# NVIDIA/nvidia-resiliency-ext

Measured on AMD Instinct MI355X. Metric: generate_report_latency_us, lower is better.
Workload: dtype f32; 1 GPU; 8 ranks x 64 sections x 10000 samples per report, ring capacity 10000, relative+individual scores, gather_on_rank0; logical_ranks_per_gpu=8, rows_per_gpu=512, exchange=none (single process)

## Files before the change

### include/nvrx_straggler.h

```cpp
#ifndef NVRX_STRAGGLER_H
#define NVRX_STRAGGLER_H

#include <stddef.h>
#include <stdint.h>

#ifdef __cplusplus
extern "C" {
#endif

#define NVRX_ABI_VERSION 2

#define NVRX_OK 0
#define NVRX_ERR_INVALID (-22)
#define NVRX_ERR_NOMEM (-12)
#define NVRX_ERR_HIP (-5)
#define NVRX_ERR_STATE (-1)
#define NVRX_ERR_RANGE (-34)
#define NVRX_ERR_TIMEOUT (-62)

#define NVRX_STATS_STRIDE 8
#define NVRX_STAT_MIN 0
#define NVRX_STAT_MAX 1
#define NVRX_STAT_MED 2
#define NVRX_STAT_AVG 3
// ... 11 lines not shown
#define NVRX_SCORE_LEN(S) (2 + 2 * (S))
#define NVRX_META_WORDS 8

typedef struct nvrx_ctx nvrx_ctx;

int nvrx_abi_version(void);
const char *nvrx_last_error(void);


int nvrx_row_stats(const float *d_samples, const uint32_t *d_counts, const uint8_t *d_kinds, int rows,
                   int row_stride, float *d_stats, void *stream);

int nvrx_score(const float *d_table, int R, int K, int S, int do_indiv, int do_rel,
               const double *thresholds, float *d_scores, uint8_t *d_flags, uint32_t *d_meta,
               uint32_t *d_done_counter, uint32_t seq, const float *d_stats_src, float *d_stats_dst,
               int stats_rows, void *stream);

#define NVRX_SCORE_ROUTE_SINGLE 1
#define NVRX_SCORE_ROUTE_ROWS 2
#define NVRX_SCORE_ROUTE_ROWS_PRE 3
#define NVRX_SCORE_ROUTE_TILE16 4
#define NVRX_SCORE_ROUTE_TILE8 5
int nvrx_score_route(int R, int K, int S, const void *d_scores, const void *d_flags);

#define NVRX_ATTR_MAX_TOP 16
#define NVRX_ATTR_SCRATCH_FLOATS(K) (33 * (size_t)(K))
#define NVRX_ATTR_WORDS(n_ranks, top_n) ((size_t)(n_ranks) * 2 * (1 + (size_t)(top_n)) * 4)
int nvrx_attribute(const float *d_table, int R, int K, int S, int first_rank, int n_ranks, int top_n, int do_indiv,
                   int do_rel, float *d_minmed_scratch, void *d_out, void *stream);

int nvrx_row_quantile(const float *d_samples, const uint32_t *d_counts, int rows, int row_stride, uint32_t q_ppm,
                      float *d_out, void *stream);
int nvrx_tail_score(const float *d_tails, const float *d_table, int R, int K, int S, int first_rank, int n_ranks,
                    float *d_colmin_scratch, float *d_out, void *stream);

int nvrx_row_onset(const float *d_samples, const uint32_t *d_counts, const uint32_t *d_starts, int rows, int row_stride,
                   uint32_t min_seg_ppm, void *d_out, void *stream);
#define NVRX_ONSET_PLANES 6
int nvrx_onset_score(const float *d_onset, const float *d_table, int R, int K, int S, int first_rank, int n_ranks,
                     float *d_colmin_scratch, float *d_out, void *stream);

#define NVRX_PERIOD_MIN_CYCLES 4
#define NVRX_PERIOD_MAX 4096
#define NVRX_PERIOD_BAR 0.95
int nvrx_row_period(const float *d_samples, const uint32_t *d_counts, const uint32_t *d_starts, int rows, int row_stride,
                    int max_period, void *d_out, void *stream);
// ... 212 lines not shown
```

### nvidia-resiliency-ext_amd/csrc/nvrx_straggler.hip

```cpp
#include <hip/hip_runtime.h>
#include <hip/hip_ext.h>

#include <algorithm>
#include <atomic>
#include <chrono>
#include <thread>
#include <cmath>
#include <cstdarg>
#include <cstdio>
#include <cstdlib>
#include <cstring>
#include <deque>
#include <mutex>
#include <string>
#include <unordered_map>
#include <utility>
#include <vector>

#include "nvrx_straggler.h"

namespace {

thread_local std::string g_err;

// ... 21 lines not shown
    g_report_clk[i] = std::chrono::duration<double, std::micro>(std::chrono::steady_clock::now().time_since_epoch()).count();
}

__device__ __forceinline__ uint32_t f2key(float f) {
    uint32_t u = __float_as_uint(f);
    return u ^ ((u >> 31) ? 0xFFFFFFFFu : 0x80000000u);
}
__device__ __forceinline__ float key2f(uint32_t k) {
    uint32_t u = (k & 0x80000000u) ? (k ^ 0x80000000u) : ~k;
    return __uint_as_float(u);
}

typedef float f32x2 __attribute__((ext_vector_type(2)));

template <int CTRL, int ROW_MASK = 0xf>
__device__ __forceinline__ uint32_t dpp(uint32_t old, uint32_t src) {
    return (uint32_t)__builtin_amdgcn_update_dpp((int)old, (int)src, CTRL, ROW_MASK, 0xf, false);
}
template <int CTRL>
__device__ __forceinline__ uint32_t dpp0(uint32_t src) {
    return (uint32_t)__builtin_amdgcn_update_dpp(0, (int)src, CTRL, 0xf, 0xf, true);
}
constexpr int DPP_QUAD_1032 = 0xb1, DPP_QUAD_2301 = 0x4e, DPP_ROW_SHR1 = 0x111, DPP_ROW_SHR2 = 0x112,
              DPP_ROW_SHR4 = 0x114, DPP_ROW_SHR8 = 0x118, DPP_BCAST15 = 0x142, DPP_BCAST31 = 0x143;

__device__ __forceinline__ uint32_t wave_min_u32(uint32_t v) {
    v = min(v, dpp<DPP_QUAD_1032>(0xFFFFFFFFu, v));
    v = min(v, dpp<DPP_QUAD_2301>(0xFFFFFFFFu, v));
    v = min(v, dpp<DPP_ROW_SHR4>(0xFFFFFFFFu, v));
    v = min(v, dpp<DPP_ROW_SHR8>(0xFFFFFFFFu, v));
    v = min(v, dpp<DPP_BCAST15>(0xFFFFFFFFu, v));
    v = min(v, dpp<DPP_BCAST31>(0xFFFFFFFFu, v));
    return (uint32_t)__builtin_amdgcn_readlane((int)v, 63);
}
__device__ __forceinline__ uint32_t wave_max_u32(uint32_t v) {
    v = max(v, dpp0<DPP_QUAD_1032>(v));
    v = max(v, dpp0<DPP_QUAD_2301>(v));
    v = max(v, dpp0<DPP_ROW_SHR4>(v));
    v = max(v, dpp0<DPP_ROW_SHR8>(v));
    v = max(v, dpp0<DPP_BCAST15>(v));
    v = max(v, dpp0<DPP_BCAST31>(v));
    return (uint32_t)__builtin_amdgcn_readlane((int)v, 63);
}
__device__ __forceinline__ uint32_t wave_sum_u32(uint32_t v) {
    v += dpp0<DPP_QUAD_1032>(v);
    v += dpp0<DPP_QUAD_2301>(v);
    v += dpp0<DPP_ROW_SHR4>(v);
// ... 1142 lines not shown
    }
}

__global__ __launch_bounds__(PEER_THREADS) void k_peer_allgather(PeerArgs a) { peer_exchange_block(a); }

constexpr int SCORE1_THREADS = 1024;
constexpr int SCORE1_RESIDENT_THREADS = 256;
constexpr int SCORE1_MAX_RANKS = 64;
constexpr size_t SCORE1_MAX_LDS = 60 * 1024;

__device__ __forceinline__ void store16_sys(void *dst, nvrx_f4 v) {
    asm volatile("global_store_dwordx4 %0, %1, off sc0 sc1" : : "v"(dst), "v"(v) : "memory");
}

__host__ __device__ inline size_t score1_lds_bytes(int R, int K, int S) {
    const size_t ks4 = (size_t)((K + S + 3) & ~3);
    const size_t nout = (size_t)R * NVRX_SCORE_LEN(S);
    return ks4 * 4 + ((nout + 3) & ~(size_t)3) * 4 + ((nout + 15) & ~(size_t)15);
}
__host__ __device__ inline size_t score1_table_lds_bytes(int R, int K, int S, int send_floats) {
    return (((size_t)R * NVRX_TABLE_LEN(K, S) + 3) & ~(size_t)3) * 4 + (((size_t)send_floats + 3) & ~(size_t)3) * 4;
}

struct GatherArgs {
    const unsigned long long *g;
    const int32_t *gid;
    float *send;
    nvrx_f4 *stats_out;
    uint32_t *err;
    int n_blocks, rows_active, rows_per_rank, local_ranks;
    float names_ok;
    uint32_t epoch;
    unsigned long long timeout_ticks;
    int poll_naps;
};

__device__ __forceinline__ float wait_granule(const unsigned long long *p, const GatherArgs &g, unsigned long long t0) {
    uint32_t spins = 0;
    for (;;) {
        const unsigned long long x = __hip_atomic_load(p, __ATOMIC_RELAXED, __HIP_MEMORY_SCOPE_AGENT);
        if ((uint32_t)(x >> 32) == g.epoch) return __uint_as_float((uint32_t)x);
        __builtin_amdgcn_s_sleep(2);
        if ((++spins & 0xFFu) == 0u && wall_clock64() - t0 > g.timeout_ticks) {
            __hip_atomic_store(g.err, g.epoch, __ATOMIC_RELAXED, __HIP_MEMORY_SCOPE_SYSTEM);
            return __builtin_nanf("");
        }
    }
}

template <int NTHR>
__global__ __launch_bounds__(NTHR) void k_score1(ScoreArgs a, int fence, PeerArgs pa, GatherArgs ga) {
    extern __shared__ __attribute__((aligned(16))) unsigned char s_raw[];

    const int K = a.K, S = a.S, KS = K + S, R = a.R;
    const int L = NVRX_TABLE_LEN(K, S);
    const int W = NVRX_SCORE_LEN(S);
    const int nout = R * W;
    const int nout4 = (nout + 3) & ~3;
    float *s_min = reinterpret_cast<float *>(s_raw);
    float *s_out = s_min + ((KS + 3) & ~3);
    uint8_t *s_fl = reinterpret_cast<uint8_t *>(s_out + nout4);
    float *s_tab = a.tab_in_lds ? reinterpret_cast<float *>(s_fl + ((nout + 15) & ~15)) : nullptr;
    float *s_send = a.tab_in_lds ? s_tab + ((R * L + 3) & ~3) : nullptr;
    const int tid = threadIdx.x;
    const float NaN = __builtin_nanf("");
    const unsigned long long t_begin = wall_clock64();
#if NVRX_TOUCH_KERNARGS
    {
        constexpr int KARG_DWORDS = (int)((sizeof(ScoreArgs) + sizeof(int) + sizeof(PeerArgs) + sizeof(GatherArgs)) / 4);
        const uint32_t __attribute__((address_space(4))) *ka =
// ... 1 lines not shown
        uint32_t touched = 0u;
#pragma unroll
        for (int d = 0; d < KARG_DWORDS; d += 16) touched ^= ka[d];
        asm volatile("" ::"s"(touched));
    }
#endif
    const int pair_r0 = tid / max(S, 1), pair_s0 = tid - pair_r0 * S;
    const int pair_dr = NTHR / max(S, 1), pair_ds = NTHR - pair_dr * S;
    const bool lds_only = ga.g && s_send;
    auto sync = [&]() {
        if (lds_only)
            asm volatile("s_waitcnt lgkmcnt(0)\n\ts_barrier" ::: "memory");
        else
            __syncthreads();
    };

    if (ga.g && s_send) {
        for (int j = tid; j < a.send_floats; j += NTHR) {
            const int col = j % L;
            s_send[j] = col < KS ? -1.0f : (col < 2 * KS ? NaN : 0.0f);
        }
        __syncthreads();
    }
    if (ga.g) {
        constexpr int CH = 8;
        const int total = ga.n_blocks * 3;
        for (int base = tid; base < total; base += NTHR * CH) {
            unsigned long long x[CH];
            int slot[CH];
            uint32_t pending = 0;
#pragma unroll
            for (int c = 0; c < CH; c++) {
                slot[c] = -1;
                const int idx = base + c * NTHR;
                if (idx < total) {
                    pending |= 1u << c;
                    const int b = idx / 3, q = idx - 3 * b;
                    const int lr = b / ga.rows_active;
                    const int gidv = ga.gid[lr * ga.rows_per_rank + (b - lr * ga.rows_active)];
                    if (gidv >= 0 && gidv < KS && (q < 2 || gidv < K)) slot[c] = lr * L + q * KS + gidv;
                }
            }
            uint32_t spins = 0;
            while (pending) {
#pragma unroll
                for (int c = 0; c < CH; c++)
                    if (pending & (1u << c)) {
// ... 9 lines not shown
                    if (!got && (spins & 0xFFu) == 0xFFu && wall_clock64() - t_begin > ga.timeout_ticks) {
                        __hip_atomic_store(ga.err, ga.epoch, __ATOMIC_RELAXED, __HIP_MEMORY_SCOPE_SYSTEM);
                        v = NaN;
                        got = true;
                    }
                    if (got) {
                        if (slot[c] >= 0) {
                            ga.send[slot[c]] = v;
                            if (s_send) s_send[slot[c]] = v;
                        }
                        pending &= ~(1u << c);
                    }
                }
                if (pending) {
                    for (int nap = 0; nap < ga.poll_naps; nap++) __builtin_amdgcn_s_sleep(1);
                    spins++;
                }
            }
        }
        for (int lr = tid; lr < ga.local_ranks; lr += NTHR) {
            ga.send[(size_t)lr * L + (L - 1)] = ga.names_ok;
            if (s_send) s_send[lr * L + (L - 1)] = ga.names_ok;
        }
        sync();
    }
    const unsigned long long t_rows = wall_clock64();
    if (pa.windows) {
        peer_exchange_block(pa, ga.g ? s_send : nullptr, s_tab);
        __syncthreads();
        if (s_tab) a.table = s_tab;
    } else if (ga.g && s_send) {
        a.table = s_send;
    }
    for (int i = tid; i < a.stats_n4; i += NTHR) {
        const float4 v = a.stats_src[i];
        store16_sys(a.stats_dst + i, nvrx_f4{v.x, v.y, v.z, v.w});
    }
    auto score_all = [&](const float *tab) {
        score_colmin(a, tab, tid, NTHR, s_min);
        if (a.meta && (tid >> 6) == NTHR / 64 - 1) score_meta(a, tab, tid & 63);
        if (tid < nout4 - nout) s_out[nout + tid] = 0.f;
        if (tid < ((nout + 15) & ~15) - nout) s_fl[nout + tid] = 0;
        sync();

        {
            int r = pair_r0, sct = pair_s0;
#pragma unroll 2
            for (int idx = tid; idx < R * S; idx += NTHR) {
                const float *__restrict__ row = tab + (size_t)r * L;
                const float med = row[K + sct];
                float si = NaN, sr = NaN;
                if (med >= 0.0f) {
                    if (a.do_indiv) si = __fdiv_rn(row[KS + K + sct], med);
                    if (a.do_rel) sr = __fdiv_rn(s_min[K + sct], med);
                }
                s_out[r * W + 2 + sct] = si;
                s_out[r * W + 2 + S + sct] = sr;
                s_fl[r * W + 2 + sct] = ((double)si < a.thr[3]) ? 1 : 0;
                s_fl[r * W + 2 + S + sct] = ((double)sr < a.thr[1]) ? 1 : 0;
                r += pair_dr;
                sct += pair_ds;
                if (sct >= S) {
                    sct -= S;
                    r++;
                }
            }
        }
        if (K == 0) {
            for (int r = tid; r < R; r += NTHR) {
                s_out[r * W] = NaN;
                s_out[r * W + 1] = NaN;
                s_fl[r * W] = 0;
                s_fl[r * W + 1] = 0;
            }
        } else {
            const int lane = tid & 63;
            for (int r = tid >> 6; r < R; r += NTHR / 64) {
                const float *__restrict__ row = tab + (size_t)r * L;
                double wi = 0.0, si = 0.0, wr = 0.0, sr = 0.0;
                uint32_t nk = 0, ncommon = 0;
                for (int k = lane; k < K; k += 64) {
                    const float medf = row[k];
                    if (!(medf >= 0.0f)) continue;
                    const double med = (double)medf;
                    const double w = (double)row[2 * KS + k];
                    nk++;
                    si += ((double)row[KS + k] / med) * w;
                    wi += w;
                    const float mm = s_min[k];
                    if (mm == mm) {
                        ncommon++;
                        sr += ((double)mm / med) * w;
                        wr += w;
                    }
                }
                wi = wave_sum_f64(wi);
                si = wave_sum_f64(si);
                wr = wave_sum_f64(wr);
                sr = wave_sum_f64(sr);
                nk = wave_sum_u32(nk);
                ncommon = wave_sum_u32(ncommon);
                if (lane == 0) {
                    const float gi = (a.do_indiv && nk > 0) ? (float)(si / wi) : NaN;
                    const float gr = (a.do_rel && ncommon > 0) ? (float)(sr / wr) : NaN;
                    s_out[r * W] = gi;
                    s_out[r * W + 1] = gr;
                    s_fl[r * W] = ((double)gi < a.thr[2]) ? 1 : 0;
                    s_fl[r * W + 1] = ((double)gr < a.thr[0]) ? 1 : 0;
                }
            }
        }
        sync();
    };
    if (s_tab && pa.windows)
        score_all(s_tab);
    else if (ga.g && s_send && !pa.windows)
        score_all(s_send);
    else
        score_all(a.table);

    const unsigned long long t_staged = wall_clock64();
    {
        const nvrx_f4 *src = reinterpret_cast<const nvrx_f4 *>(s_out);
        nvrx_f4 *dst = reinterpret_cast<nvrx_f4 *>(a.scores);
        for (int i = tid; i < nout4 / 4; i += NTHR) store16_sys(dst + i, src[i]);
        if (a.flags) {
            const nvrx_f4 *fsrc = reinterpret_cast<const nvrx_f4 *>(s_fl);
            nvrx_f4 *fdst = reinterpret_cast<nvrx_f4 *>(a.flags);
            for (int i = tid; i < (nout + 15) / 16; i += NTHR) store16_sys(fdst + i, fsrc[i]);
        }
    }
    asm volatile("s_waitcnt vmcnt(0)" ::: "memory");
    __syncthreads();
    const bool publish = a.meta && a.done_counter;
    if (tid == 0 && publish) {
        if (fence) {
            __builtin_amdgcn_fence(__ATOMIC_RELEASE, "");
            asm volatile("s_waitcnt vmcnt(0)" ::: "memory");
        }
        if (!(ga.g && ga.stats_out))
            __hip_atomic_store(&a.meta[5], a.seq, __ATOMIC_RELAXED, __HIP_MEMORY_SCOPE_SYSTEM);
        __hip_atomic_store(&a.meta[6], (uint32_t)(t_rows - t_begin), __ATOMIC_RELAXED, __HIP_MEMORY_SCOPE_SYSTEM);
        __hip_atomic_store(&a.meta[7], (uint32_t)min(wall_clock64() - t_rows, 0xFFFFull) | ((uint32_t)min(t_staged - t_rows, 0xFFFFull) << 16),
                           __ATOMIC_RELAXED, __HIP_MEMORY_SCOPE_SYSTEM);
// ... 75 lines not shown

constexpr int score_single_wg_enabled() { return 1; }
int score_fence_enabled() {
    static int v = -1;
    if (v < 0) {
        const char *e = getenv("NVRX_DEBUG_SCORE_FENCE");
        if (e && *e) {
            v = atoi(e) != 0 ? 1 : 0;
        } else {
            int dev = 0;
            hipDeviceProp_t prop;
            v = 1;
            if (hipGetDevice(&dev) == hipSuccess && hipGetDeviceProperties(&prop, dev) == hipSuccess &&
                (strncmp(prop.gcnArchName, "gfx950", 6) == 0 || strncmp(prop.gcnArchName, "gfx942", 6) == 0))
                v = 0;
        }
    }
    return v;
}

int resident_scorer_mode_from_env() {
    const char *e = getenv("NVRX_DEBUG_RESIDENT_SCORER");
    const int v = e ? atoi(e) : 1;
    return (v < 0 || v > 2) ? 1 : v;
}
constexpr int poll_naps_from_env() {
    return 4;
}

constexpr int peer_prologue_enabled() { return 1; }

struct ScoreScratch {
    float *ptr = nullptr;
    size_t elems = 0;
};
std::mutex g_scratch_mu;
std::unordered_map<void *, ScoreScratch> g_scratch_by_stream;

}

struct EventPair {
    hipEvent_t start = nullptr;
    hipEvent_t end = nullptr;
};

struct StageBuf {
    uint32_t *h_counts = nullptr;
// ... 335 lines not shown
    Epilogue ep{};
    return launch_row_stats(d_samples, d_counts, d_kinds, rows, row_stride, d_stats, ep, as_stream(stream));
}

static bool score_fits_single_wg(int R, int K, int S, const float *d_scores, const uint8_t *d_flags) {
    return R <= SCORE1_MAX_RANKS && score1_lds_bytes(R, K, S) <= SCORE1_MAX_LDS &&
           (reinterpret_cast<uintptr_t>(d_scores) & 15u) == 0 && (reinterpret_cast<uintptr_t>(d_flags) & 15u) == 0 &&
           score_single_wg_enabled();
}

constexpr size_t SCORE_ROWS_MAX_LDS = 48 * 1024;

static int score_route(int R, int K, int S, const float *d_scores, const uint8_t *d_flags) {
    if (score_fits_single_wg(R, K, S, d_scores, d_flags)) return NVRX_SCORE_ROUTE_SINGLE;
    if (R <= 64 && (size_t)(K + S) * sizeof(float) <= SCORE_ROWS_MAX_LDS) return NVRX_SCORE_ROUTE_ROWS;
    const bool aligned = ((reinterpret_cast<uintptr_t>(d_scores) | reinterpret_cast<uintptr_t>(d_flags)) & 15u) == 0;
    if (aligned && R > 64) {
        if (score_tile_lds_bytes(16, S) <= TILE_MAX_LDS) return NVRX_SCORE_ROUTE_TILE16;
        if (score_tile_lds_bytes(8, S) <= TILE_MAX_LDS) return NVRX_SCORE_ROUTE_TILE8;
    }
    return NVRX_SCORE_ROUTE_ROWS_PRE;
}

static int score_launch(const float *d_table, int R, int K, int S, int do_indiv, int do_rel, const double *thresholds,
                        float *d_scores, uint8_t *d_flags, uint32_t *d_meta, uint32_t *d_done_counter, uint32_t seq,
                        const float *d_stats_src, float *d_stats_dst, int stats_rows, void *stream, const PeerArgs *pa,
                        const GatherArgs *ga = nullptr) {
    if (R <= 0 || K < 0 || S < 0) return fail(NVRX_ERR_INVALID, "bad table shape R=%d K=%d S=%d", R, K, S);
    if (!d_table || !d_scores) return fail(NVRX_ERR_INVALID, "null device pointer");
    hipStream_t st = as_stream(stream);
    ScoreArgs a{};
    a.table = d_table;
    a.R = R;
    a.K = K;
    a.S = S;
    a.do_indiv = do_indiv;
    a.do_rel = do_rel;
    for (int i = 0; i < 4; i++) a.thr[i] = thresholds ? thresholds[i] : 0.75;
    a.scores = d_scores;
    a.flags = d_flags;
    a.meta = d_meta;
    a.done_counter = d_meta ? d_done_counter : nullptr;
    a.seq = seq;
    if (d_stats_src && d_stats_dst && stats_rows > 0) {
        a.stats_src = reinterpret_cast<const float4 *>(d_stats_src);
        a.stats_dst = reinterpret_cast<float4 *>(d_stats_dst);
        a.stats_n4 = stats_rows * (NVRX_STATS_STRIDE / 4);
    }
    const int KS = K + S;
    const int route = score_route(R, K, S, d_scores, d_flags);
    if (route == NVRX_SCORE_ROUTE_SINGLE) {
        PeerArgs none{};
        GatherArgs nog{};
        size_t lds1 = score1_lds_bytes(R, K, S);
        if (ga || pa) {
            const int send_floats = pa ? pa->count : R * NVRX_TABLE_LEN(K, S);
            const size_t extra = score1_table_lds_bytes(R, K, S, send_floats);
            if (lds1 + extra <= SCORE1_MAX_LDS) {
                a.tab_in_lds = 1;
                a.send_floats = send_floats;
                lds1 += extra;
            }
        }
        if (ga) {
            a.stats_n4 = 0;
            hipLaunchKernelGGL(k_score1<SCORE1_RESIDENT_THREADS>, dim3(1), dim3(SCORE1_RESIDENT_THREADS), lds1, st, a,
                               score_fence_enabled(), pa ? *pa : none, *ga);
        } else {
            report_clk(7);
            hipLaunchKernelGGL(k_score1<SCORE1_THREADS>, dim3(1), dim3(SCORE1_THREADS), lds1, st, a, score_fence_enabled(),
                               pa ? *pa : none, nog);
        }
        HIP_TRY(hipGetLastError());
        return NVRX_OK;
    }
    if (ga) return fail(NVRX_ERR_STATE, "the resident scorer needs the single-workgroup score kernel");
    if (pa) return fail(NVRX_ERR_STATE, "the exchange prologue needs the single-workgroup score kernel");
    if (route != NVRX_SCORE_ROUTE_ROWS) {
        const int chunks = std::max(1, std::min(COLMIN_MAX_CHUNKS, (R + 63) / 64));
        const int rows_per_chunk = (R + chunks - 1) / chunks;
        const size_t need = (size_t)KS * (size_t)(chunks + 1);
        float *scratch = nullptr;
        {
            std::lock_guard<std::mutex> lk(g_scratch_mu);
            ScoreScratch &sc = g_scratch_by_stream[stream];
            if (sc.elems < need) {
                if (sc.ptr) HIP_TRY(hipFree(sc.ptr));
                sc = ScoreScratch{};
                HIP_TRY(hipMalloc(reinterpret_cast<void **>(&sc.ptr), std::max<size_t>(need, 1024) * sizeof(float)));
                sc.elems = std::max<size_t>(need, 1024);
// ... 15 lines not shown
        hipLaunchKernelGGL(k_score, dim3(R), dim3(SCORE_THREADS), (size_t)KS * sizeof(float), st, a);
        break;
    case NVRX_SCORE_ROUTE_ROWS_PRE:
        hipLaunchKernelGGL(k_score, dim3(R), dim3(SCORE_THREADS), 0, st, a);
        break;
    case NVRX_SCORE_ROUTE_TILE16:
    case NVRX_SCORE_ROUTE_TILE8: {
        const int tile_ranks = route == NVRX_SCORE_ROUTE_TILE16 ? 16 : 8;
        hipLaunchKernelGGL(k_score_tile, dim3((R + tile_ranks - 1) / tile_ranks), dim3(TILE_THREADS),
                           score_tile_lds_bytes(tile_ranks, S), st, a, tile_ranks);
        break;
    }
    default:
        return fail(NVRX_ERR_STATE, "no score kernel for route %d", route);
    }
    HIP_TRY(hipGetLastError());
    return NVRX_OK;
}

int nvrx_score_route(int R, int K, int S, const void *d_scores, const void *d_flags) {
    if (R <= 0 || K < 0 || S < 0) return fail(NVRX_ERR_INVALID, "bad table shape R=%d K=%d S=%d", R, K, S);
    return score_route(R, K, S, static_cast<const float *>(d_scores), static_cast<const uint8_t *>(d_flags));
}

int nvrx_score(const float *d_table, int R, int K, int S, int do_indiv, int do_rel, const double *thresholds,
               float *d_scores, uint8_t *d_flags, uint32_t *d_meta, uint32_t *d_done_counter, uint32_t seq,
               const float *d_stats_src, float *d_stats_dst, int stats_rows, void *stream) {
    return score_launch(d_table, R, K, S, do_indiv, do_rel, thresholds, d_scores, d_flags, d_meta, d_done_counter, seq,
                        d_stats_src, d_stats_dst, stats_rows, stream, nullptr);
}

int nvrx_send_init(float *d_send, int rows, int K, int S, void *stream) {
    if (!d_send || rows <= 0 || K < 0 || S < 0) return fail(NVRX_ERR_INVALID, "bad arguments");
    const size_t n = (size_t)rows * NVRX_TABLE_LEN(K, S);
    hipLaunchKernelGGL(k_send_init, dim3((unsigned)((n + 255) / 256)), dim3(256), 0, as_stream(stream), d_send, rows, K, S);
    HIP_TRY(hipGetLastError());
    return NVRX_OK;
}

int nvrx_ctx_create(int device, int local_ranks, int rows_per_rank, int ring_cap, nvrx_ctx **out) {
    if (!out) return fail(NVRX_ERR_INVALID, "out is null");
    *out = nullptr;
    if (local_ranks <= 0 || rows_per_rank <= 0 || ring_cap <= 0) return fail(NVRX_ERR_INVALID, "sizes must be positive");
    if (ring_cap > NVRX_MAX_RING_CAP) return fail(NVRX_ERR_RANGE, "ring_cap %d > %d", ring_cap, NVRX_MAX_RING_CAP);
    if ((long long)local_ranks * rows_per_rank > NVRX_MAX_ROWS) return fail(NVRX_ERR_RANGE, "too many rows");
    int ndev = 0;
// ... 858 lines not shown
        }
    }
    if (!rehomed && d->order_after_enabled && d->order_after_stream != stream) {
        std::lock_guard<std::mutex> lk(ctx->mu);
        HIP_TRY(hipEventRecord(ctx->order_ev, as_stream(d->order_after_stream)));
        HIP_TRY(hipStreamWaitEvent(as_stream(stream), ctx->order_ev, 0));
    }
    report_clk(1);
    if (d->R > 64) {
        std::lock_guard<std::mutex> lk(ctx->mu);
        if (std::find(ctx->report_streams.begin(), ctx->report_streams.end(), as_stream(stream)) == ctx->report_streams.end())
            ctx->report_streams.push_back(as_stream(stream));
    }
    const int rows_launch = (d->rows_active > 0 ? d->rows_active : ctx->rows_per_rank) * ctx->local_ranks;
    const bool peer_route = exchanging && d->allgather_fn == reinterpret_cast<void *>(&nvrx_peer_allgather) && peer_prologue_enabled();
    bool cross_stream = rehomed || (d->order_after_enabled && d->order_after_stream != stream);
    {
        std::lock_guard<std::mutex> lk(ctx->mu);
        cross_stream = cross_stream || !ctx->stamp_streams.empty();
    }
    const int rmode = ctx->resident_mode;
    const bool resident = d->resident && d->h_seq_word && !d->guard_rings && (!exchanging || peer_route) && rows_launch > 0 &&
                          score_fits_single_wg(d->R, d->K, d->S, d->d_scores, d->d_flags) &&
                          (rmode == 2 || (rmode == 1 && !cross_stream));
    if (resident) {
        {
            std::lock_guard<std::mutex> lk(ctx->mu);
            HIP_TRY(hipSetDevice(ctx->device));
            if (!ctx->score_stream) {
                bool high = true;
                const char *pe = getenv("NVRX_STREAM_PRIORITY");
                if (pe && *pe) {
                    high = !(pe[0] == 'n' || pe[0] == 'N' || pe[0] == '0' || pe[0] == 'o' || pe[0] == 'O');
                } else {
                    for (const char *var : {"WORLD_SIZE", "SLURM_NTASKS", "OMPI_COMM_WORLD_SIZE", "PMI_SIZE"}) {
                        const char *v = getenv(var);
                        if (!v || !*v) continue;
                        const long n = strtol(v, nullptr, 10);
                        if (n > 1) high = false;
                        if (n > 1 || strcmp(var, "WORLD_SIZE") == 0) break;
                    }
                }
                if (high) {
                    int least = 0, greatest = 0;
                    HIP_TRY(hipDeviceGetStreamPriorityRange(&least, &greatest));
                    HIP_TRY(hipStreamCreateWithPriority(&ctx->score_stream, hipStreamNonBlocking, greatest));
                } else {
// ... 6 lines not shown
                int orc = order_after_stamps(ctx, as_stream(stream), ctx->score_stream);
                if (orc) return orc;
            }
        }
        ctx->gran_epoch = (ctx->gran_epoch % 0x7FFFFFFFu) + 1u;
        unsigned long long *slice = ctx->d_rowg + (size_t)(ctx->gran_epoch & 1u) * (size_t)ctx->rows * ROW_GRANULES;
        int rc2 = report_local_impl(ctx, d->d_stats, d->d_send, d->K, d->S, d->names_ok, d->rows_active, stream, slice,
                                    ctx->gran_epoch);
        if (rc2) return rc2;
        GatherArgs ga{};
        ga.g = slice;
        ga.gid = ctx->d_gid;
        ga.send = d->d_send;
        ga.stats_out = (d->d_stats_dst && d->stats_rows > 0) ? reinterpret_cast<nvrx_f4 *>(d->d_stats_dst) : nullptr;
        ga.err = ctx->d_gather_err;
        ga.n_blocks = rows_launch;
        ga.rows_active = d->rows_active > 0 ? d->rows_active : ctx->rows_per_rank;
        ga.rows_per_rank = ctx->rows_per_rank;
        ga.local_ranks = ctx->local_ranks;
        ga.names_ok = d->names_ok ? 1.0f : 0.0f;
        ga.epoch = ctx->gran_epoch;
        ga.timeout_ticks = (unsigned long long)((d->timeout_s > 0.0 ? d->timeout_s : 1e9) * 1e3 * (double)ctx->wall_khz);
        ga.poll_naps = ctx->poll_naps;
        PeerArgs pa{};
        if (peer_route) {
            rc2 = peer_fill_args(static_cast<nvrx_peer *>(d->comm), d->d_send, d->d_table, (size_t)d->send_count, &pa);
            if (rc2) return rc2;
        }
        d->seq = (d->seq % 0x7FFFFFFFu) + 1u;
        rc2 = score_launch(exchanging ? d->d_table : d->d_send, d->R, d->K, d->S, d->do_indiv, d->do_rel, d->thresholds,
                           d->d_scores, d->d_flags, d->d_meta, d->d_done_counter, d->seq, nullptr, nullptr, 0,
                           ctx->score_stream, peer_route ? &pa : nullptr, &ga);
        if (rc2) return rc2;
        ctx->attr_desc = d, ctx->attr_stream = ctx->score_stream;
        report_clk(4);
        report_clk(5);
        rc2 = nvrx_poll_u32(d->h_seq_word, d->seq, d->timeout_s > 0.0 ? d->timeout_s : 1e30);
        report_clk(6);
        if (rc2) return rc2;
        if (*static_cast<volatile uint32_t *>(ctx->h_gather_err) == ctx->gran_epoch)
            return fail(NVRX_ERR_TIMEOUT, "the score kernel gave up waiting for the statistics kernel's rows (epoch %u)", ctx->gran_epoch);
        if (as_stream(stream) == ctx->default_stream) {
            std::lock_guard<std::mutex> lk(ctx->mu);
            ctx->side_work = false;
            ctx->async_on_ctx = false;
        }
// ... 396 lines not shown
```

### nvidia-resiliency-ext_amd/nvrx_straggler/_native.py

```python
from __future__ import annotations

import ctypes
import os
import threading
from ctypes import POINTER, c_char_p, c_double, c_float, c_int, c_int32, c_size_t, c_uint32, c_uint64, c_void_p

_LIB_NAME = "libnvrx_straggler_hip.so"
_LIB_PATH = os.path.join(os.environ.get("NVRX_DEBUG_LIB_DIR") or os.path.join(os.path.dirname(os.path.abspath(__file__)), "lib"), _LIB_NAME)

NVRX_ABI_VERSION = 2
STATS_STRIDE = 8
STAT_MIN, STAT_MAX, STAT_MED, STAT_AVG, STAT_STD, STAT_NUM, STAT_WEIGHT = range(7)
KIND_SECTION, KIND_KERNEL = 0, 1
MAX_RING_CAP = 65536
META_WORDS = 8
ERR_TIMEOUT = -62
ERR_RANGE = -34
ERR_INVALID = -22
ERR_STATE = -1
ATTR_MAX_TOP = 16
TAIL_Q_PPM_MIN, TAIL_Q_PPM_MAX = 500000, 999999
ROUTE_SINGLE, ROUTE_ROWS, ROUTE_ROWS_PRE, ROUTE_TILE16, ROUTE_TILE8 = 1, 2, 3, 4, 5
ROBUST_MAX_RANKS = 65536
PEER_MAX_GROUPS = 4096
# ... 32 lines not shown
        ("h_seq_word", c_void_p), ("timeout_s", c_double),
        ("order_after_stream", c_void_p), ("order_after_enabled", c_int32), ("resident", c_int32), ("prev_settled", c_int32), ("guard_rings", c_int32),
    ]


class WindowDesc(ctypes.Structure):

    _fields_ = [
        ("kt_sync", c_void_p), ("kt_hold", c_void_p), ("kt_counter", c_void_p), ("kt_patience_s", c_double),
        ("kt_rows_known", ctypes.c_uint64), ("kt_keys_without_row", ctypes.c_uint64),
        ("rows_used", c_int32), ("asynchronous", c_int32), ("harvest_regions", c_int32), ("out_names_ok", c_int32),
    ]


WINDOW_MISS, WINDOW_NAMES = 1, 2

SYMBOLS = [
    ("nvrx_abi_version", c_int, []),
    ("nvrx_last_error", c_char_p, []),
    ("nvrx_row_stats", c_int, [c_void_p, c_void_p, c_void_p, c_int, c_int, c_void_p, c_void_p]),
    ("nvrx_score", c_int, [c_void_p, c_int, c_int, c_int, c_int, c_int, POINTER(c_double), c_void_p, c_void_p, c_void_p,
                           c_void_p, c_uint32, c_void_p, c_void_p, c_int, c_void_p]),
    ("nvrx_score_route", c_int, [c_int, c_int, c_int, c_void_p, c_void_p]),
    ("nvrx_attribute", c_int, [c_void_p, c_int, c_int, c_int, c_int, c_int, c_int, c_int, c_int, c_void_p, c_void_p, c_void_p]),
    ("nvrx_row_quantile", c_int, [c_void_p, c_void_p, c_int, c_int, c_uint32, c_void_p, c_void_p]),
    ("nvrx_tail_score", c_int, [c_void_p, c_void_p, c_int, c_int, c_int, c_int, c_int, c_void_p, c_void_p, c_void_p]),
    ("nvrx_row_onset", c_int, [c_void_p, c_void_p, c_void_p, c_int, c_int, c_uint32, c_void_p, c_void_p]),
    ("nvrx_onset_score", c_int, [c_void_p, c_void_p, c_int, c_int, c_int, c_int, c_int, c_void_p, c_void_p, c_void_p]),
    ("nvrx_row_period", c_int, [c_void_p, c_void_p, c_void_p, c_int, c_int, c_int, c_void_p, c_void_p]),
    ("nvrx_period_score", c_int, [c_void_p, c_void_p, c_int, c_int, c_int, c_int, c_int, c_void_p, c_void_p, c_void_p]),
    ("nvrx_row_episode", c_int, [c_void_p, c_void_p, c_void_p, c_int, c_int, c_uint32, c_void_p, c_void_p]),
    ("nvrx_episode_score", c_int, [c_void_p, c_void_p, c_int, c_int, c_int, c_int, c_int, c_void_p, c_void_p, c_void_p]),
    ("nvrx_robust_score", c_int, [c_void_p, c_int, c_int, c_int, c_int, c_int, c_int, c_float, c_void_p, c_void_p]),
    ("nvrx_peer_score", c_int, [c_void_p, c_int, c_int, c_int, c_void_p, c_int, c_int, c_int, c_int, c_void_p, c_void_p]),
    ("nvrx_pace_score", c_int, [c_void_p, c_int, c_int, c_int, c_int, c_int, c_int, c_void_p, c_void_p]),
    ("nvrx_pace_group_score", c_int, [c_void_p, c_int, c_int, c_int, c_void_p, c_int, c_int, c_int, c_int, c_int, c_int, c_void_p,
                                      c_void_p]),
    ("nvrx_node_score", c_int, [c_void_p, c_int, c_int, c_int, c_void_p, c_int, c_int, c_int, c_int, c_int, c_int, c_void_p,
                                c_void_p]),
    ("nvrx_score_history", c_int, [c_void_p, c_int, c_int, c_int, c_int, c_void_p, c_int, c_int, c_uint64, POINTER(c_double),
                                   c_void_p, c_void_p]),
    ("nvrx_score_trend", c_int, [c_void_p, c_int, c_int, c_int, c_int, c_uint64, c_void_p, c_void_p]),
    ("nvrx_peer_history", c_int, [c_void_p, c_int, c_int, c_void_p, c_int, c_int, c_uint64, POINTER(c_double), c_void_p,
                                  c_void_p]),
    ("nvrx_peer_trend", c_int, [c_void_p, c_int, c_int, c_int, c_int, c_uint64, c_void_p, c_void_p]),
    ("nvrx_slack_score", c_int, [c_void_p, c_void_p, c_int, c_int, c_int, c_int, c_void_p, c_void_p]),
# ... 278 lines not shown
```

Measured before the change: 26.74 us.

## Add column-ordered resident scorer that scores sections as granules arrive

Adds a column-wise body to the resident single-workgroup scorer. Each thread owns (rank, section) columns, polls its granules, writes them to the send buffer, and computes individual and relative section scores as soon as a whole column has landed. The column min is reduced with DPP group minima. This overlaps scoring with waiting on the gather instead of running a separate colmin/score pass after all rows arrive. In exchange it uses more LDS and a more complex polling loop, and it only applies when R*K*S fit within the pair/thread limits.

```diff
diff --git a/include/nvrx_straggler.h b/include/nvrx_straggler.h
--- a/include/nvrx_straggler.h
+++ b/include/nvrx_straggler.h
@@ -57,6 +57,10 @@
 #define NVRX_SCORE_ROUTE_TILE16 4
 #define NVRX_SCORE_ROUTE_TILE8 5
 int nvrx_score_route(int R, int K, int S, const void *d_scores, const void *d_flags);
+
+#define NVRX_RESIDENT_BODY_FLAT 0
+#define NVRX_RESIDENT_BODY_COLUMNS 1
+int nvrx_score_resident_body(int R, int K, int S, int rows);
 
 #define NVRX_ATTR_MAX_TOP 16
 #define NVRX_ATTR_SCRATCH_FLOATS(K) (33 * (size_t)(K))
diff --git a/nvidia-resiliency-ext_amd/csrc/nvrx_straggler.hip b/nvidia-resiliency-ext_amd/csrc/nvrx_straggler.hip
--- a/nvidia-resiliency-ext_amd/csrc/nvrx_straggler.hip
+++ b/nvidia-resiliency-ext_amd/csrc/nvrx_straggler.hip
@@ -67,7 +67,8 @@
     return (uint32_t)__builtin_amdgcn_update_dpp(0, (int)src, CTRL, 0xf, 0xf, true);
 }
 constexpr int DPP_QUAD_1032 = 0xb1, DPP_QUAD_2301 = 0x4e, DPP_ROW_SHR1 = 0x111, DPP_ROW_SHR2 = 0x112,
-              DPP_ROW_SHR4 = 0x114, DPP_ROW_SHR8 = 0x118, DPP_BCAST15 = 0x142, DPP_BCAST31 = 0x143;
+              DPP_ROW_SHR4 = 0x114, DPP_ROW_SHR8 = 0x118, DPP_BCAST15 = 0x142, DPP_BCAST31 = 0x143,
+              DPP_ROW_MIRROR = 0x140, DPP_ROW_HALF_MIRROR = 0x141;
 
 __device__ __forceinline__ uint32_t wave_min_u32(uint32_t v) {
     v = min(v, dpp<DPP_QUAD_1032>(0xFFFFFFFFu, v));
@@ -1256,6 +1257,10 @@
     return (((size_t)R * NVRX_TABLE_LEN(K, S) + 3) & ~(size_t)3) * 4 + (((size_t)send_floats + 3) & ~(size_t)3) * 4;
 }
 
+__host__ __device__ inline size_t score1_columns_lds_bytes(int R, int K, int S) {
+    return (((size_t)R * (size_t)(K + S) + 3) & ~(size_t)3) * 4 + (SCORE1_RESIDENT_THREADS / 64) * sizeof(unsigned long long);
+}
+
 struct GatherArgs {
     const unsigned long long *g;
     const int32_t *gid;
@@ -1267,6 +1272,7 @@
     uint32_t epoch;
     unsigned long long timeout_ticks;
     int poll_naps;
+    int col_rp;
 };
 
 __device__ __forceinline__ float wait_granule(const unsigned long long *p, const GatherArgs &g, unsigned long long t0) {
@@ -1280,6 +1286,232 @@
             return __builtin_nanf("");
         }
     }
+}
+
+template <int NTHR>
+__device__ __forceinline__ void score1_gpu_scores(const ScoreArgs &a, const float *tab, const float *s_min, float *s_out,
+                                                  uint8_t *s_fl, int tid) {
+    const int K = a.K, KS = a.K + a.S, R = a.R;
+    const int L = NVRX_TABLE_LEN(a.K, a.S), W = NVRX_SCORE_LEN(a.S);
+    const float NaN = __builtin_nanf("");
+    const int lane = tid & 63;
+    for (int r = tid >> 6; r < R; r += NTHR / 64) {
+        const float *__restrict__ row = tab + (size_t)r * L;
+        double wi = 0.0, si = 0.0, wr = 0.0, sr = 0.0;
+        uint32_t nk = 0, ncommon = 0;
+        for (int k = lane; k < K; k += 64) {
+            const float medf = row[k];
+            if (!(medf >= 0.0f)) continue;
+            const double med = (double)medf;
+            const double w = (double)row[2 * KS + k];
+            nk++;
+            si += ((double)row[KS + k] / med) * w;
+            wi += w;
+            const float mm = s_min[k];
+            if (mm == mm) {
+                ncommon++;
+                sr += ((double)mm / med) * w;
+                wr += w;
+            }
+        }
+        wi = wave_sum_f64(wi);
+        si = wave_sum_f64(si);
+        wr = wave_sum_f64(wr);
+        sr = wave_sum_f64(sr);
+        nk = wave_sum_u32(nk);
+        ncommon = wave_sum_u32(ncommon);
+        if (lane == 0) {
+            const float gi = (a.do_indiv && nk > 0) ? (float)(si / wi) : NaN;
+            const float gr = (a.do_rel && ncommon > 0) ? (float)(sr / wr) : NaN;
+            s_out[r * W] = gi;
+            s_out[r * W + 1] = gr;
+            s_fl[r * W] = ((double)gi < a.thr[2]) ? 1 : 0;
+            s_fl[r * W + 1] = ((double)gr < a.thr[0]) ? 1 : 0;
+        }
+    }
+}
+
+#ifdef NVRX_TAIL_CLOCKS
+__device__ unsigned long long g_tail_clk[8];
+#define NVRX_TAIL(i)                                            \
+    do {                                                        \
+        if (threadIdx.x == 0) g_tail_clk[i] = wall_clock64(); \
+    } while (0)
+#else
+#define NVRX_TAIL(i) \
+    do {             \
+    } while (0)
+#endif
+
+constexpr int SCORE1_COL_PAIRS = 2;
+constexpr int SCORE1_COL_MAX_BLOCKS = 8192;
+
+__device__ __forceinline__ float group_min_first(float v, int lane, int Rp) {
+    auto step = [&](float o, int d) {
+        return (lane & d) ? (v < o ? v : o) : (o < v ? o : v);
+    };
+    if (Rp > 1) v = step(__uint_as_float(dpp0<DPP_QUAD_1032>(__float_as_uint(v))), 1);
+    if (Rp > 2) v = step(__uint_as_float(dpp0<DPP_QUAD_2301>(__float_as_uint(v))), 2);
+    if (Rp > 4) v = step(__uint_as_float(dpp0<DPP_ROW_HALF_MIRROR>(__float_as_uint(v))), 4);
+    if (Rp > 8) v = step(__uint_as_float(dpp0<DPP_ROW_MIRROR>(__float_as_uint(v))), 8);
+    if (Rp > 16) v = step(__shfl_xor(v, 16), 16);
+    if (Rp > 32) v = step(__shfl_xor(v, 32), 32);
+    return v;
+}
+
+template <int NTHR>
+__device__ __forceinline__ unsigned long long score1_columns(const ScoreArgs &a, const GatherArgs &ga, float *s_min,
+                                                             float *s_out, uint8_t *s_fl, float *s_send, int32_t *s_inv,
+                                                             unsigned long long *s_clk, unsigned long long t_begin) {
+    constexpr int P = SCORE1_COL_PAIRS;
+    const int K = a.K, S = a.S, KS = K + S, R = a.R;
+    const int L = NVRX_TABLE_LEN(K, S), W = NVRX_SCORE_LEN(S);
+    const int nout = R * W, nout4 = (nout + 3) & ~3;
+    const int tid = threadIdx.x, lane = tid & 63;
+    const float NaN = __builtin_nanf("");
+    const int Rp = ga.col_rp, sh = __ffs(Rp) - 1;
+    const int r = tid & (Rp - 1);
+    const bool real = r < R;
+    const unsigned long long gmask = (Rp == 64 ? ~0ull : (1ull << Rp) - 1ull) << (lane & ~(Rp - 1));
+
+    for (int i = tid; i < R * KS; i += NTHR) s_inv[i] = -1;
+    if (tid < nout4 - nout) s_out[nout + tid] = 0.f;
+    if (tid < ((nout + 15) & ~15) - nout) s_fl[nout + tid] = 0;
+    if (K == 0)
+        for (int q = tid; q < R; q += NTHR) {
+            s_out[q * W] = NaN;
+            s_out[q * W + 1] = NaN;
+            s_fl[q * W] = 0;
+            s_fl[q * W + 1] = 0;
+        }
+    for (int lr = tid; lr < ga.local_ranks; lr += NTHR) {
+        ga.send[(size_t)lr * L + (L - 1)] = ga.names_ok;
+        s_send[lr * L + (L - 1)] = ga.names_ok;
+    }
+    __syncthreads();
+    uint32_t no_slot = 0;
+    for (int b = tid, k = 0; b < ga.n_blocks; b += NTHR, k++) {
+        const int lr = b / ga.rows_active;
+        const int gidv = ga.gid[lr * ga.rows_per_rank + (b - lr * ga.rows_active)];
+        if (gidv >= 0 && gidv < KS && lr < R)
+            s_inv[lr * KS + gidv] = b;
+        else
+            no_slot |= 1u << k;
+    }
+    __syncthreads();
+    if (a.meta && (tid >> 6) == NTHR / 64 - 1) score_meta(a, s_send, lane);
+
+    double thr_ind = a.thr[3], thr_rel = a.thr[1];
+    asm volatile("" : "+v"(thr_ind), "+v"(thr_rel));
+    int blk[P];
+    float med[P], ref[P];
+    uint32_t pend = 0, scored = 0, cdone = 0;
+#pragma unroll
+    for (int i = 0; i < P; i++) {
+        const int j = (tid >> sh) + i * (NTHR >> sh);
+        blk[i] = -1;
+        med[i] = real ? -1.0f : INFINITY;
+        ref[i] = NaN;
+        if (j >= KS) {
+            scored |= 1u << i;
+            cdone |= 1u << i;
+        } else if (!real) {
+            scored |= 1u << i;
+        } else {
+            blk[i] = s_inv[r * KS + j];
+            if (blk[i] >= 0) pend |= (j < K ? 7u : 3u) << (3 * i);
+        }
+    }
+
+    uint32_t spins = 0;
+    unsigned long long t_seen = 0;
+    unsigned long long x[P][3] = {};
+    for (bool first = true;; first = false) {
+#pragma unroll
+        for (int i = 0; i < P; i++)
+#pragma unroll
+            for (int q = 0; q < 3; q++)
+                if (pend & (1u << (3 * i + q)))
+                    x[i][q] = __hip_atomic_load(ga.g + (size_t)blk[i] * ROW_GRANULES + q, __ATOMIC_RELAXED, __HIP_MEMORY_SCOPE_AGENT);
+        uint32_t got = 0;
+#pragma unroll
+        for (int i = 0; i < P; i++)
+#pragma unroll
+            for (int q = 0; q < 3; q++)
+                if ((uint32_t)(x[i][q] >> 32) == ga.epoch) got |= 1u << (3 * i + q);
+        got &= pend;
+        uint32_t gone = 0;
+        if (pend && (spins & 0xFFu) == 0xFFu && wall_clock64() - t_begin > ga.timeout_ticks) {
+            gone = pend & ~got;
+            if (gone) __hip_atomic_store(ga.err, ga.epoch, __ATOMIC_RELAXED, __HIP_MEMORY_SCOPE_SYSTEM);
+        }
+        if (!first && __ballot((got | gone) != 0u) == 0ull) {
+            for (int nap = 0; nap < ga.poll_naps; nap++) __builtin_amdgcn_s_sleep(1);
+            spins++;
+            continue;
+        }
+#pragma unroll
+        for (int i = 0; i < P; i++) {
+            const int j = (tid >> sh) + i * (NTHR >> sh);
+#pragma unroll
+            for (int q = 0; q < 3; q++) {
+                if (!((got | gone) & (1u << (3 * i + q)))) continue;
+                const float v = (gone & (1u << (3 * i + q))) ? NaN : __uint_as_float((uint32_t)x[i][q]);
+                const int slot = r * L + q * KS + j;
+                ga.send[slot] = v;
+                s_send[slot] = v;
+                if (q == 0) med[i] = v;
+                if (q == 1) ref[i] = v;
+            }
+            if (!(scored & (1u << i)) && (((pend & ~(got | gone)) >> (3 * i)) & 7u) == 0u) {
+                scored |= 1u << i;
+                if (j >= K) {
+                    const float si = (med[i] >= 0.0f && a.do_indiv) ? __fdiv_rn(ref[i], med[i]) : NaN;
+                    s_out[r * W + 2 + (j - K)] = si;
+                    s_fl[r * W + 2 + (j - K)] = ((double)si < thr_ind) ? 1 : 0;
+                }
+            }
+        }
+        pend &= ~(got | gone);
+        if (!t_seen && __ballot(pend != 0u) == 0ull) t_seen = wall_clock64();
+#pragma unroll
+        for (int i = 0; i < P; i++) {
+            const unsigned long long have = __ballot((scored >> i) & 1u);
+            const bool now = !(cdone & (1u << i)) && (have & gmask) == gmask;
+            if (__ballot(now) == 0ull) continue;
+            float m = group_min_first(med[i] == med[i] ? med[i] : INFINITY, lane, Rp);
+            m = m >= 0.0f ? m : NaN;
+            if (now) {
+                cdone |= 1u << i;
+                if (real) {
+                    const int j = (tid >> sh) + i * (NTHR >> sh);
+                    if (r == 0) s_min[j] = m;
+                    if (j >= K) {
+                        const float sr = (med[i] >= 0.0f && a.do_rel) ? __fdiv_rn(m, med[i]) : NaN;
+                        s_out[r * W + 2 + S + (j - K)] = sr;
+                        s_fl[r * W + 2 + S + (j - K)] = ((double)sr < thr_rel) ? 1 : 0;
+                    }
+                }
+            }
+        }
+        if (__ballot(cdone != (1u << P) - 1u) == 0ull) break;
+        if (__ballot(pend != 0u) != 0ull) spins++;
+    }
+    if (lane == 0) s_clk[tid >> 6] = t_seen;
+    for (int k = 0; no_slot; k++, no_slot >>= 1)
+        if (no_slot & 1u)
+            for (int q = 0; q < 3; q++) (void)wait_granule(ga.g + (size_t)(tid + k * NTHR) * ROW_GRANULES + q, ga, t_begin);
+    NVRX_TAIL(0);
+    asm volatile("s_waitcnt lgkmcnt(0)\n\ts_barrier" ::: "memory");
+    NVRX_TAIL(1);
+    unsigned long long t_rows = 0;
+    for (int w = 0; w < NTHR / 64; w++) t_rows = max(t_rows, s_clk[w]);
+
+    if (K > 0) {
+        score1_gpu_scores<NTHR>(a, s_send, s_min, s_out, s_fl, tid);
+        asm volatile("s_waitcnt lgkmcnt(0)\n\ts_barrier" ::: "memory");
+    }
+    return t_rows;
 }
 
 template <int NTHR>
@@ -1327,7 +1559,15 @@
         }
         __syncthreads();
     }
-    if (ga.g) {
+    const bool by_columns = NTHR == SCORE1_RESIDENT_THREADS && ga.col_rp != 0;
+    unsigned long long t_rows = 0;
+    if (by_columns) {
+        if constexpr (NTHR == SCORE1_RESIDENT_THREADS) {
+            int32_t *s_inv = reinterpret_cast<int32_t *>(s_send + ((a.send_floats + 3) & ~3));
+            unsigned long long *s_clk = reinterpret_cast<unsigned long long *>(s_inv + ((R * KS + 3) & ~3));
+            t_rows = score1_columns<NTHR>(a, ga, s_min, s_out, s_fl, s_send, s_inv, s_clk, t_begin);
+        }
+    } else if (ga.g) {
         constexpr int CH = 8;
         const int total = ga.n_blocks * 3;
         for (int base = tid; base < total; base += NTHR * CH) {
@@ -1383,9 +1623,11 @@
             ga.send[(size_t)lr * L + (L - 1)] = ga.names_ok;
             if (s_send) s_send[lr * L + (L - 1)] = ga.names_ok;
         }
+        NVRX_TAIL(0);
         sync();
-    }
-    const unsigned long long t_rows = wall_clock64();
+        NVRX_TAIL(1);
+    }
+    if (!by_columns) t_rows = wall_clock64();
     if (pa.windows) {
         peer_exchange_block(pa, ga.g ? s_send : nullptr, s_tab);
         __syncthreads();
@@ -1399,10 +1641,12 @@
     }
     auto score_all = [&](const float *tab) {
         score_colmin(a, tab, tid, NTHR, s_min);
+        NVRX_TAIL(2);
         if (a.meta && (tid >> 6) == NTHR / 64 - 1) score_meta(a, tab, tid & 63);
         if (tid < nout4 - nout) s_out[nout + tid] = 0.f;
         if (tid < ((nout + 15) & ~15) - nout) s_fl[nout + tid] = 0;
         sync();
+        NVRX_TAIL(3);
 
         {
             int r = pair_r0, sct = pair_s0;
@@ -1427,6 +1671,7 @@
                 }
             }
         }
+        NVRX_TAIL(4);
         if (K == 0) {
             for (int r = tid; r < R; r += NTHR) {
                 s_out[r * W] = NaN;
@@ -1435,45 +1680,13 @@
                 s_fl[r * W + 1] = 0;
             }
         } else {
-            const int lane = tid & 63;
-            for (int r = tid >> 6; r < R; r += NTHR / 64) {
-                const float *__restrict__ row = tab + (size_t)r * L;
-                double wi = 0.0, si = 0.0, wr = 0.0, sr = 0.0;
-                uint32_t nk = 0, ncommon = 0;
-                for (int k = lane; k < K; k += 64) {
-                    const float medf = row[k];
-                    if (!(medf >= 0.0f)) continue;
-                    const double med = (double)medf;
-                    const double w = (double)row[2 * KS + k];
-                    nk++;
-                    si += ((double)row[KS + k] / med) * w;
-                    wi += w;
-                    const float mm = s_min[k];
-                    if (mm == mm) {
-                        ncommon++;
-                        sr += ((double)mm / med) * w;
-                        wr += w;
-                    }
-                }
-                wi = wave_sum_f64(wi);
-                si = wave_sum_f64(si);
-                wr = wave_sum_f64(wr);
-                sr = wave_sum_f64(sr);
-                nk = wave_sum_u32(nk);
-                ncommon = wave_sum_u32(ncommon);
-                if (lane == 0) {
-                    const float gi = (a.do_indiv && nk > 0) ? (float)(si / wi) : NaN;
-                    const float gr = (a.do_rel && ncommon > 0) ? (float)(sr / wr) : NaN;
-                    s_out[r * W] = gi;
-                    s_out[r * W + 1] = gr;
-                    s_fl[r * W] = ((double)gi < a.thr[2]) ? 1 : 0;
-                    s_fl[r * W + 1] = ((double)gr < a.thr[0]) ? 1 : 0;
-                }
-            }
+            score1_gpu_scores<NTHR>(a, tab, s_min, s_out, s_fl, tid);
         }
         sync();
     };
-    if (s_tab && pa.windows)
+    if (by_columns)
+        ;
+    else if (s_tab && pa.windows)
         score_all(s_tab);
     else if (ga.g && s_send && !pa.windows)
         score_all(s_send);
@@ -1481,6 +1694,7 @@
         score_all(a.table);
 
     const unsigned long long t_staged = wall_clock64();
+    NVRX_TAIL(5);
     {
         const nvrx_f4 *src = reinterpret_cast<const nvrx_f4 *>(s_out);
         nvrx_f4 *dst = reinterpret_cast<nvrx_f4 *>(a.scores);
@@ -1602,7 +1816,7 @@
 int resident_scorer_mode_from_env() {
     const char *e = getenv("NVRX_DEBUG_RESIDENT_SCORER");
     const int v = e ? atoi(e) : 1;
-    return (v < 0 || v > 2) ? 1 : v;
+    return (v < 0 || v > 3) ? 1 : v;
 }
 constexpr int poll_naps_from_env() {
     return 4;
@@ -1984,6 +2198,19 @@
     return NVRX_SCORE_ROUTE_ROWS_PRE;
 }
 
+static int score_resident_rp(int R, int K, int S, int rows) {
+    const long long KS = (long long)K + S;
+    if (R > SCORE1_MAX_RANKS || KS == 0) return 0;
+    int Rp = 1;
+    while (Rp < R) Rp <<= 1;
+    if (KS * Rp > (long long)SCORE1_COL_PAIRS * SCORE1_RESIDENT_THREADS) return 0;
+    if (rows > SCORE1_COL_MAX_BLOCKS) return 0;
+    const size_t lds = score1_lds_bytes(R, K, S) + score1_table_lds_bytes(R, K, S, R * NVRX_TABLE_LEN(K, S));
+    if (lds > SCORE1_MAX_LDS) return 0;
+    if (lds + score1_columns_lds_bytes(R, K, S) > SCORE1_MAX_LDS) return 0;
+    return Rp;
+}
+
 static int score_launch(const float *d_table, int R, int K, int S, int do_indiv, int do_rel, const double *thresholds,
                         float *d_scores, uint8_t *d_flags, uint32_t *d_meta, uint32_t *d_done_counter, uint32_t seq,
                         const float *d_stats_src, float *d_stats_dst, int stats_rows, void *stream, const PeerArgs *pa,
@@ -2026,8 +2253,11 @@
         }
         if (ga) {
             a.stats_n4 = 0;
+            GatherArgs g = *ga;
+            g.col_rp = (g.col_rp && !pa && a.tab_in_lds && g.local_ranks == R) ? score_resident_rp(R, K, S, g.n_blocks) : 0;
+            if (g.col_rp) lds1 += score1_columns_lds_bytes(R, K, S);
             hipLaunchKernelGGL(k_score1<SCORE1_RESIDENT_THREADS>, dim3(1), dim3(SCORE1_RESIDENT_THREADS), lds1, st, a,
-                               score_fence_enabled(), pa ? *pa : none, *ga);
+                               score_fence_enabled(), pa ? *pa : none, g);
         } else {
             report_clk(7);
             hipLaunchKernelGGL(k_score1<SCORE1_THREADS>, dim3(1), dim3(SCORE1_THREADS), lds1, st, a, score_fence_enabled(),
@@ -2089,6 +2319,18 @@
     if (R <= 0 || K < 0 || S < 0) return fail(NVRX_ERR_INVALID, "bad table shape R=%d K=%d S=%d", R, K, S);
     return score_route(R, K, S, static_cast<const float *>(d_scores), static_cast<const uint8_t *>(d_flags));
 }
+
+int nvrx_score_resident_body(int R, int K, int S, int rows) {
+    if (R <= 0 || K < 0 || S < 0 || rows < 0) return fail(NVRX_ERR_INVALID, "bad table shape R=%d K=%d S=%d rows=%d", R, K, S, rows);
+    return score_resident_rp(R, K, S, rows) ? NVRX_RESIDENT_BODY_COLUMNS : NVRX_RESIDENT_BODY_FLAT;
+}
+
+#ifdef NVRX_TAIL_CLOCKS
+int nvrx_debug_tail_clocks(unsigned long long *out) {
+    HIP_TRY(hipMemcpyFromSymbol(out, HIP_SYMBOL(g_tail_clk), sizeof(g_tail_clk)));
+    return NVRX_OK;
+}
+#endif
 
 int nvrx_score(const float *d_table, int R, int K, int S, int do_indiv, int do_rel, const double *thresholds,
                float *d_scores, uint8_t *d_flags, uint32_t *d_meta, uint32_t *d_done_counter, uint32_t seq,
@@ -2993,7 +3235,7 @@
     const int rmode = ctx->resident_mode;
     const bool resident = d->resident && d->h_seq_word && !d->guard_rings && (!exchanging || peer_route) && rows_launch > 0 &&
                           score_fits_single_wg(d->R, d->K, d->S, d->d_scores, d->d_flags) &&
-                          (rmode == 2 || (rmode == 1 && !cross_stream));
+                          (rmode >= 2 || (rmode == 1 && !cross_stream));
     if (resident) {
         {
             std::lock_guard<std::mutex> lk(ctx->mu);
@@ -3046,6 +3288,7 @@
         ga.epoch = ctx->gran_epoch;
         ga.timeout_ticks = (unsigned long long)((d->timeout_s > 0.0 ? d->timeout_s : 1e9) * 1e3 * (double)ctx->wall_khz);
         ga.poll_naps = ctx->poll_naps;
+        ga.col_rp = rmode == 3 ? 0 : 1;
         PeerArgs pa{};
         if (peer_route) {
             rc2 = peer_fill_args(static_cast<nvrx_peer *>(d->comm), d->d_send, d->d_table, (size_t)d->send_count, &pa);
diff --git a/nvidia-resiliency-ext_amd/nvrx_straggler/_native.py b/nvidia-resiliency-ext_amd/nvrx_straggler/_native.py
--- a/nvidia-resiliency-ext_amd/nvrx_straggler/_native.py
+++ b/nvidia-resiliency-ext_amd/nvrx_straggler/_native.py
@@ -78,6 +78,7 @@
     ("nvrx_score", c_int, [c_void_p, c_int, c_int, c_int, c_int, c_int, POINTER(c_double), c_void_p, c_void_p, c_void_p,
                            c_void_p, c_uint32, c_void_p, c_void_p, c_int, c_void_p]),
     ("nvrx_score_route", c_int, [c_int, c_int, c_int, c_void_p, c_void_p]),
+    ("nvrx_score_resident_body", c_int, [c_int, c_int, c_int, c_int]),
     ("nvrx_attribute", c_int, [c_void_p, c_int, c_int, c_int, c_int, c_int, c_int, c_int, c_int, c_void_p, c_void_p, c_void_p]),
     ("nvrx_row_quantile", c_int, [c_void_p, c_void_p, c_int, c_int, c_uint32, c_void_p, c_void_p]),
     ("nvrx_tail_score", c_int, [c_void_p, c_void_p, c_int, c_int, c_int, c_int, c_int, c_void_p, c_void_p, c_void_p]),
```

Result: slower. 28.70 us (+7.3%).
